# erthward/geonomics

Hardware: AMD Instinct MI355X
Metric: individual-timesteps/sec (higher is better)
Workload: dtype u64

## Files before the change

geonomics_amd/_native.py:

```python
import ctypes as C
import os

import numpy as np

_HERE = os.path.dirname(os.path.abspath(__file__))
LIB_PATH = os.environ.get('GNX_LIB') or os.path.join(_HERE, 'libgnxhip.so')

DIST = {'lognormal': 0, 'wald': 1, 'levy': 2}
MATE_UNIFORM, MATE_NEAREST, MATE_INVERSE = 0, 1, 2
SURF_NONE, SURF_MIXTURE, SURF_UNIMODAL = 0, 1, 2
(F_X, F_Y, F_AGE, F_SEX, F_ID, F_E, F_Z, F_FIT, F_GROW, F_GENO) = range(10)
(R_N, R_NPAIRS, R_K, R_D, R_COUNTS) = range(5)
KERNELS = ['move', 'sort', 'permute', 'find_mates', 'pairs', 'offspring',
           'crossover', 'phenotype', 'density', 'death', 'compact', 'crossover_tail']

EXPORTS = [
    'gnx_create', 'gnx_destroy', 'gnx_last_error', 'gnx_words_per_hom', 'gnx_blocks_per_hom',
    'gnx_set_stream', 'gnx_synchronize', 'gnx_upload_rasters',
    'gnx_upload_layer', 'gnx_set_species_params', 'gnx_upload_population',
    'gnx_init_population', 'gnx_set_recomb_paths', 'gnx_set_trait',
    'gnx_set_dominance', 'gnx_set_deleterious', 'gnx_upload_genomes',
    'gnx_assign_genomes', 'gnx_set_z', 'gnx_age', 'gnx_move',
    'gnx_pop_dynamics', 'gnx_pop_dynamics_mate', 'gnx_pop_dynamics_die',
    'gnx_set_z_range', 'gnx_step', 'gnx_counts', 'gnx_step_index',
# ... 377 lines not shown
        self._chk(self.lib.gnx_tile2_vt_counts(self.h, _ptr(cnt, C.c_int64)))
        return cnt

    def tile2_vt_bases(self, bases):
        b = _arr(bases, np.int64)
        assert b.size == 64
        self._chk(self.lib.gnx_tile2_vt_bases(self.h, _ptr(b, C.c_int64)))

    def step_begin(self, burn):
        self._chk(self.lib.gnx_step_begin(self.h, int(bool(burn))))

    def step_mid(self, burn, with_selection):
        self._chk(self.lib.gnx_step_mid(self.h, int(bool(burn)), int(bool(with_selection))))

    def step_end(self, burn):
        self._chk(self.lib.gnx_step_end(self.h, int(bool(burn))))

    def counts(self):
        n, b, d = C.c_int64(), C.c_int64(), C.c_int64()
        self._chk(self.lib.gnx_counts(self.h, C.byref(n), C.byref(b), C.byref(d)))
        return n.value, b.value, d.value

    def totals(self):
        out = np.zeros(6, np.int64)
        self._chk(self.lib.gnx_totals(self.h, _ptr(out, C.c_int64)))
        return dict(zip(('steps', 'ind_steps', 'births', 'deaths', 'xo_births', 'dd_steps'),
                        (int(v) for v in out)))

    def reset_totals(self):
        self._chk(self.lib.gnx_reset_totals(self.h))

    PATH_COUNTS = ('lazy_mortalities', 'xo_launch_p2', 'xo_flush', 'jobs_lanes_256',
                   'jobs_lanes_512', 'sort_hist_gather', 'gc_with_pending_xo', 'make_dense',
                   'moves_ahead')

    def path_counts(self):
        out = np.zeros(len(self.PATH_COUNTS), np.int64)
        n = self.lib.gnx_path_counts(self.h, _ptr(out, C.c_int64), len(out))
        assert n == len(out), 'gnx_path_counts: the library has %d counters' % n
        return dict(zip(self.PATH_COUNTS, (int(v) for v in out)))

    def reset_path_counts(self):
        self._chk(self.lib.gnx_reset_path_counts(self.h))

    @property
    def N(self):
        return self.counts()[0]

    @property
    def step_index(self):
        return self.lib.gnx_step_index(self.h)

    @step_index.setter
    def step_index(self, v):
        self._chk(self.lib.gnx_set_step_index(self.h, C.c_int64(int(v))))

    def synchronize(self):
        self._chk(self.lib.gnx_synchronize(self.h))

    def set_defer_crossover(self, on):
        self._chk(self.lib.gnx_set_defer_crossover(self.h, int(bool(on))))

    def set_crossover_overlap(self, mode):
        self._chk(self.lib.gnx_set_crossover_overlap(self.h, int(mode)))

    def debug_halves(self):
        out = np.zeros(6, np.int64)
# ... 1295 lines not shown
```

geonomics_amd/csrc/gnx_api.hip:

```cpp
#include <cmath>
#include <cstdarg>
#include <algorithm>
#include <atomic>
#include <chrono>
#include "gnx_internal.h"
#include "gnx_rng.h"
#include "gnx_compact.h"

static thread_local char g_err[1024] = "";

void gnx_set_error(const char* fmt, ...) {
  va_list ap;
  va_start(ap, fmt);
  vsnprintf(g_err, sizeof(g_err), fmt, ap);
  va_end(ap);
}

extern "C" const char* gnx_last_error(void) { return g_err; }

extern "C" int gnx_words_per_hom(int32_t L) {
  int w = (L + 63) / 64;
  return ((w + 15) / 16) * 16;
}

// ... 375 lines not shown
  GNXCHK(dalloc(&h->req_px, cap));
  GNXCHK(dalloc(&h->req_py, cap));
  GNXCHK(dalloc(&h->req_count, 1));
  h->blk_stride = (int)((cap + 1023) / 1024) + 2;
  GNXCHK(dalloc(&h->blk_cnt, (size_t)3 * h->blk_stride));
  GNXCHK(dalloc(&h->blk_off, (size_t)3 * h->blk_stride));
  GNXCHK(dalloc(&h->cnt_dev, 8));
  GNXCHK(dalloc(&h->tickets, 8));
  GNXCHK(dalloc(&h->nmax2, 2));
  HIPCHK(hipMemset(h->nmax2, 0, 2 * sizeof(unsigned long long)));
  HIPCHK(hipEventCreateWithFlags(&h->ev_pairs, gnx_order_event_flags()));
  HIPCHK(hipEventCreateWithFlags(&h->ev_latP, gnx_order_event_flags()));
  HIPCHK(hipEventCreateWithFlags(&h->ev_perm, gnx_order_event_flags()));
  HIPCHK(hipEventCreateWithFlags(&h->ev_binsN, gnx_order_event_flags()));
  HIPCHK(hipMemset(h->tickets, 0, 8 * sizeof(unsigned int)));
  HIPCHK(hipHostMalloc((void**)&h->h_pin, 32 * sizeof(int64_t),
                       hipHostMallocCoherent | hipHostMallocMapped));
  memset(h->h_pin, 0, 32 * sizeof(int64_t));
  HIPCHK(hipHostGetDevicePointer((void**)&h->h_pin_dev, h->h_pin, 0));
  if (cfg->L > 0) {
    for (int k = 0; k < 2; ++k) {
      HIPCHK(hipMalloc(&h->jobs[k], (size_t)cap * 2 * h->NB * 16));
      HIPCHK(hipMalloc(&h->jobs_bp[k], (size_t)cap * 2 * h->NB * 8));
      GNXCHK(dalloc(&h->n_jobs_dev[k], 1));
      HIPCHK(hipEventCreateWithFlags(&h->ev_xo_done[k], gnx_order_event_flags()));
      HIPCHK(hipEventCreateWithFlags(&h->ev_xo_wide[k], gnx_order_event_flags()));
    }
    HIPCHK(hipEventCreateWithFlags(&h->ev_jobs, gnx_order_event_flags()));
  }
  HIPCHK(hipEventCreateWithFlags(&h->ev_counts, hipEventDisableTiming));
  h->xo_launch_late = h->xo_launch_late_default = cap > gnx_dd_max_cap();
  h->compact_fill = gnx_env_int("GNX_COMPACT_FILL", 1) != 0;
  h->permute_split = gnx_env_int("GNX_PERMUTE_SPLIT", 1) != 0;
  *out = h;
  return 0;
}

extern "C" void gnx_destroy(gnx_state* h) {
  if (!h) return;
  host_marks_report();
  if (gnx_host_times() && g_host_steps > 0)
    fprintf(stderr, "[gnx host times] %lld steps: %.1f us/step in gnx_step, %.1f us of it waiting for counts\n",
            g_host_steps, 1e6 * g_host_step_s / g_host_steps, 1e6 * g_host_wait_s / g_host_steps);
  (void)gnx_xo_launch_pending(h);
  (void)hipStreamSynchronize(h->stream);
  gnx_dd_destroy(h);
  (void)gnx_comm_free(h);
  {
    void* vt[] = {h->vt_cls, h->vt_scls, h->vt_blk_nz, h->vt_rank, h->vt_pblk, h->vt_blk_cnt, h->vt_blk_off, h->vt_count, h->vt_base};
    for (void* q : vt)
      if (q) (void)hipFree(q);
  }
  if (h->stream2) (void)hipStreamSynchronize(h->stream2);
  if (h->stream3) (void)hipStreamSynchronize(h->stream3);
  for (int k = 0; k < 2; ++k) {
    (void)hipFree(h->jobs[k]);
    (void)hipFree(h->jobs_bp[k]);
    (void)hipFree(h->n_jobs_dev[k]);
    if (h->ev_xo_done[k]) (void)hipEventDestroy(h->ev_xo_done[k]);
    if (h->ev_xo_wide[k]) (void)hipEventDestroy(h->ev_xo_wide[k]);
  }
  if (h->ev_jobs) (void)hipEventDestroy(h->ev_jobs);
  if (h->ev_counts) (void)hipEventDestroy(h->ev_counts);
  for (int k = 0; k < 2; ++k) {
    free_soa(&h->soa[k]);
    (void)hipFree(h->key[k]);
// ... 580 lines not shown
  bool count;
  explicit GnxStepTimer(bool c) : count(c) {}
  ~GnxStepTimer() {
    if (gnx_host_times()) {
      g_host_step_s += std::chrono::duration<double>(std::chrono::steady_clock::now() - t0).count();
      if (count) ++g_host_steps;
    }
  }
};

extern "C" int gnx_step_begin(gnx_state* h, int32_t burn) {
  GNXCHK(need_params(h));
  GNXCHK(check_recomb_ready(h, burn != 0));
  GnxStepTimer timer(true);
  if (h->mort_wait || h->pairs_wait) {
    gnx_set_error("gnx_step_begin: the previous step of this handle was not finished (gnx_step_end)");
    return 1;
  }
  h->tot[0] += 1;
  h->tot[1] += h->N - h->n_ghost;
  h->last_xo_births = 0;
  h->step_burn = burn != 0;
  h->tile2_mode = false;
  if (h->moved_ahead) {
    GNXCHK(gnx_move_ahead_join(h));
  } else if (h->sp.move) {
    h->move_writes_keys = h->sp.mating_radius >= 0;
    int rc = gnx_l_move(h, true, nullptr, nullptr, nullptr, nullptr, true);
    h->move_writes_keys = false;
    GNXCHK(rc);
  } else {
    GNXCHK(gnx_l_age(h));
  }
  GNXCHK(gnx_l_sort_by_cell(h, true));
  int rc_pairs = gnx_l_find_pairs_enqueue(h, nullptr, true);
  GNXCHK(gnx_wait_permute_rest(h));
  return rc_pairs;
}

extern "C" int gnx_step_mid(gnx_state* h, int32_t burn, int32_t with_selection) {
  GnxStepTimer timer(false);
  int64_t P = 0, B = 0;
  GNXCHK(gnx_l_find_pairs_finish(h, &P));
  if (P > 0 && !h->spl_P.valid)
    GNXCHK(gnx_l_density(h, P, h->mid_x, h->mid_y, &h->spl_P, nullptr));
  GNXCHK(gnx_l_mate(h, burn != 0, false, 0, &B));
  h->last_births = B;
  GNXCHK(gnx_l_density_N(h));
  GNXCHK(gnx_l_death_probs(h, with_selection != 0 && !burn));
  return gnx_l_mortality_enqueue(h, nullptr);
}

extern "C" int gnx_step_end(gnx_state* h, int32_t burn) {
  GnxStepTimer timer(false);
  int64_t D = 0;
  GNXCHK(gnx_l_mortality_finish(h, &D));
  h->last_deaths = D;
  h->step += 1;
  h->tot[2] += h->last_births;
  h->tot[3] += h->last_deaths;
  if (!burn) h->tot[4] += h->last_xo_births;
  return 0;
}

extern "C" int gnx_step(gnx_state* h, int32_t burn, int32_t with_selection) {
  GNXCHK(gnx_step_begin(h, burn));
  GNXCHK(gnx_step_mid(h, burn, with_selection));
  return gnx_step_end(h, burn);
// ... 518 lines not shown
```

geonomics_amd/csrc/gnx_internal.h:

```cpp
#pragma once
#include <cstring>
#include <cstdint>
#include <cstdio>
#include <cstdlib>
#include <string>
#include <vector>
#include <utility>
#include <hip/hip_runtime.h>
#include "../../include/gnx_hip.h"
#include "gnx_half.h"

#define GNX_MAX_TRAITS 16
#define GNX_MAX_LAYERS 16
#define GNX_DISP_ATTEMPTS 8
#define GNX_SPARSE_MAX_BP 24

void gnx_set_error(const char* fmt, ...);

static inline int gnx_env_int(const char* name, int dflt) {
  const char* v = getenv(name);
  return v ? atoi(v) : dflt;
}
static inline int64_t gnx_dd_max_cap() {
  static const int64_t v = getenv("GNX_DD_MAX_CAP") ? atoll(getenv("GNX_DD_MAX_CAP")) : 600000;
// ... 181 lines not shown
  const int lane = threadIdx.x & 63;
  int idx = -1;
  while (todo) {
    const int leader = __ffsll((long long)todo) - 1;
    const int d = __shfl(dest, leader);
    const unsigned long long same = __ballot(dest == d);
    int base = 0;
    if (lane == leader) base = atomicAdd(&counts[d], (int)__popcll(same));
    base = __shfl(base, leader);
    if (dest == d) idx = base + (int)__popcll(same & ((1ull << lane) - 1ull));
    todo &= ~same;
  }
  return idx;
}
__device__ __forceinline__ int gnx_route_dest(const RouteGeo& g, int k, int orow, int oc, int cx, int cy) {
  if (k == 4) return (orow * g.C + oc) != g.me ? orow * g.C + oc : -1;
  const int rr = orow + k / 3 - 1, cc = oc + k % 3 - 1;
  if (rr >= 0 && rr < g.R && cc >= 0 && cc < g.C && cx >= g.cx0[cc] && cx <= g.cx1[cc] &&
      cy >= g.cy0[rr] && cy <= g.cy1[rr])
    return rr * g.C + cc;
  return -1;
}
#endif
enum {
  GNX_PC_LAZY_MORT = 0,
  GNX_PC_XO_P2,
  GNX_PC_XO_FLUSH,
  GNX_PC_JOBS_256,
  GNX_PC_JOBS_512,
  GNX_PC_SORT_GATHER,
  GNX_PC_GC_PENDING_XO,
  GNX_PC_MAKE_DENSE,
  GNX_PC_MOVE_AHEAD,
  GNX_PC_COUNT
};

struct gnx_state {
  gnx_config cfg{};
  gnx_species_params sp{};
  bool have_sp = false;
  hipStream_t stream = nullptr;
  hipStream_t stream2 = nullptr;
  bool xo_pending = false;
  bool own_stream = false;
  int W64 = 0;
  int64_t N = 0;
  int64_t max_id = -1;
  int64_t step = 0;
  int64_t last_births = 0, last_deaths = 0;
  int64_t tot[6]{};
  int64_t pc[GNX_PC_COUNT]{};
  int64_t n_ghost = 0;

  GnxSoA soa[2]{};
  int cur = 0;

  uint64_t* G = nullptr;
  int row_spread = 1;
  int32_t* free_rows = nullptr;
  int64_t n_free = 0;
  int32_t* hmap = nullptr;
  uint8_t* half_mark = nullptr;
  int32_t* half_free = nullptr;
  int32_t* half_top = nullptr;
  int64_t half_free_est = 0;
  int64_t gc_runs = 0;
// ... 231 lines not shown
  hipEvent_t ev_perm_rest = nullptr;
  bool fb_pending = false;
  const float *fbp_x = nullptr, *fbp_y = nullptr;
  int64_t fbp_N = 0;
  hipEvent_t ev_alive = nullptr;
  int32_t* fill_cnt = nullptr;
  hipEvent_t ev_fill = nullptr;
  int64_t fill_guess = 0;
  uint32_t* cell32 = nullptr;
  uint32_t* keyk[2]{};
  int32_t* valk[2]{};
  void* os_scratch = nullptr;
  uint32_t* os_ktmp = nullptr;
  int32_t* os_vtmp = nullptr;
  int32_t* ord_cnt = nullptr;
  int32_t* ord_off = nullptr;
  hipEvent_t ev_ord = nullptr;
  bool ord_inflight = false;
  bool keys_ordmode = false;
  bool keys_fresh = false;
  bool hist_fresh = false;
  bool holes = false;
  int64_t holes_N = 0;
  RouteGeo* route_geo_dev = nullptr;
  uint64_t route_geo_epoch = 0;
  bool move_counts_routes = false;
  bool move_counted_routes = false;
  bool tile_lazy_ok = false;
  int64_t holes_flagged = 0;
  bool eager_move = false;
  bool move_ahead_ok = false;
  bool moved_ahead = false;
  hipEvent_t ev_moved = nullptr;
  bool e_stale = false;
  bool move_writes_keys = false;
  int n_bin_blocks = 0;
  double* nodes = nullptr;
  double* K_over = nullptr;
  unsigned long long* nmax_bits = nullptr;
  double* p_death = nullptr;
  double* d_cell = nullptr;
  uint8_t* dead_in = nullptr;
  int32_t* counts_rast[2]{};
  int counts_cur = 0;
  bool counts_init = false;
  double* red = nullptr;

  int32_t* blk_cnt = nullptr;
  int32_t* blk_off = nullptr;
  int blk_stride = 0;
  int32_t* cnt_dev = nullptr;
  unsigned int* tickets = nullptr;

  int64_t* h_pin = nullptr;
  int64_t* h_pin_dev = nullptr;
  int64_t pin_seq = 0;
  void* h_stage = nullptr;
  size_t h_stage_bytes = 0;

  void* tile_comm = nullptr;
  GnxDD* dd = nullptr;
  GnxDDRec* dd_ring = nullptr;
  GnxDDRec* dd_ring_dev = nullptr;
  bool dd_active = false;
  int64_t dd_seq = 0;
  int64_t dd_seen = 0;
// ... 27 lines not shown
int gnx_half_reserve(gnx_state* h, int64_t blocks);
int gnx_gc(gnx_state* h);
static inline const int32_t* gnx_alias_bp(const gnx_state* h) {
  return (h->alias_xo && h->sparse_paths) ? h->bp_off : nullptr;
}
static inline const int32_t* gnx_alias_loci(const gnx_state* h) {
  return (h->alias_xo && h->sparse_paths) ? h->bp_loci : nullptr;
}

int gnx_publish(gnx_state* h, int slot, const int32_t* a, const int32_t* b = nullptr,
                const int32_t* c = nullptr, const int32_t* d = nullptr);

void gnx_time_begin(gnx_state* h, int kernel = -1);
void gnx_time_end(gnx_state* h, int kernel, double bytes);

int gnx_h2d(gnx_state* h, void* dst, const void* src, size_t bytes);
int gnx_d2h(gnx_state* h, void* dst, const void* src, size_t bytes);

int gnx_l_init_population(gnx_state* h, int64_t N);
int gnx_l_gather_e(gnx_state* h, int64_t first, int64_t n);
int gnx_l_age(gnx_state* h);
int gnx_l_move(gnx_state* h, bool inc_age, const float* inj_theta, const float* inj_dist,
               float* out_theta, float* out_dist, bool apply);
int gnx_l_move_ahead(gnx_state* h, int64_t N);
int gnx_move_ahead_join(gnx_state* h);
int gnx_l_sort_by_cell(gnx_state* h, bool split_rest = false);
int gnx_wait_permute_rest(gnx_state* h);
int gnx_permute_rest_launch(gnx_state* h);
int gnx_l_find_pairs(gnx_state* h, const uint8_t* d_keep, int64_t* n_pairs_out,
                     bool with_density = false);
int gnx_l_find_pairs_enqueue(gnx_state* h, const uint8_t* d_keep, bool with_density);
int gnx_l_find_pairs_finish(gnx_state* h, int64_t* n_pairs_out);
int gnx_l_births(gnx_state* h, int64_t* births_out);
int gnx_l_pair_cls(gnx_state* h, int64_t P, bool local);
int gnx_vt_buffers(gnx_state* h);
int gnx_l_mate(gnx_state* h, bool burn, bool inject, int64_t B_inject, int64_t* births_out,
               int64_t id_base = -1, bool tiled = false);
int gnx_l_dispersal_inject(gnx_state* h, int64_t B, int A, const float* d_mx, const float* d_my,
                           const float* d_theta, const float* d_dist, float* d_ox, float* d_oy,
                           int32_t* d_used);
int gnx_l_crossover_all(gnx_state* h, int64_t first_slot, int64_t B);
int gnx_l_crossover_requests(gnx_state* h, int64_t first_slot, int64_t n_req);
int gnx_l_crossover_pending(gnx_state* h, int64_t first_slot, int64_t B);
int gnx_l_crossover_survivors(gnx_state* h, int64_t first_slot, int64_t B, const int32_t* d_alive,
                              const int32_t* d_scan);
int gnx_xo_join(gnx_state* h);
int gnx_xo_flush_deferred(gnx_state* h);
int gnx_xo_launch_pending(gnx_state* h, int site = GNX_PC_XO_FLUSH);
int gnx_xo_wait_inflight(gnx_state* h);
int gnx_xo_prepare_jobs(gnx_state* h, int32_t** zero);
int gnx_xo_wait_wide(gnx_state* h);
double gnx_xo_bytes_per_birth(const gnx_state* h);
int gnx_l_rebuild_sel(gnx_state* h);
int gnx_l_path_sel(gnx_state* h);
int gnx_l_tb_from_rows(gnx_state* h, int64_t first, int64_t n, const int32_t* d_list,
                       const int64_t* d_slots, bool join = true);
int gnx_l_newborn_tb(gnx_state* h, int64_t first_slot, int64_t B);
int gnx_l_phenotype(gnx_state* h, int64_t first_slot, int64_t n, const int32_t* d_list = nullptr);
int gnx_l_assign_genomes(gnx_state* h, const int32_t* d_n_per_site);
int gnx_l_mutate(gnx_state* h, int n, const int64_t* d_slot, const int32_t* d_locus,
                 const uint8_t* d_hom);
int gnx_l_density(gnx_state* h, int64_t n, const float* d_x, const float* d_y, GnxSpline* spl,
                  const double* d_nodes_override, const int32_t* n_dev = nullptr);
struct GnxSetWords {
  int32_t* dst = nullptr;
  int32_t v[4] = {0, 0, 0, 0};
};
struct GnxPubWords {
  int n1 = 0;
  const int32_t* src1 = nullptr;
  int32_t* host1 = nullptr;
  int n2 = 0;
  const int32_t* src2 = nullptr;
  int32_t* host2 = nullptr;
};
int gnx_l_bins(gnx_state* h, int64_t n, const float* d_x, const float* d_y, const uint8_t* d_ghost,
               int32_t* d_bins, const int32_t* n_dev = nullptr, const GnxSetWords* sw = nullptr);
int gnx_l_spline(gnx_state* h, const int32_t* d_bins, GnxSpline* spl,
                 const double* d_nodes_override);
int gnx_l_spline_z(gnx_state* h, const int32_t* d_bins, GnxSpline* spl,
                   const double* d_nodes_override, bool housekeeping);
int gnx_l_raster(gnx_state* h, int which, double* d_out);
int gnx_l_density_N(gnx_state* h);
int gnx_l_lattice_P_async(gnx_state* h, int64_t n_max);
int gnx_bins_adults_launch(gnx_state* h);
void gnx_bins_adults_drop(gnx_state* h);
int gnx_l_bins_adults_async(gnx_state* h, const float* d_x, const float* d_y, int64_t N);
int gnx_wait_latP(gnx_state* h);
bool gnx_fused_bins(const gnx_state* h);
int gnx_l_death_probs(gnx_state* h, bool with_selection);
int gnx_l_mortality(gnx_state* h, const uint8_t* d_dead_inject, int64_t* deaths_out);
int gnx_l_mortality_enqueue(gnx_state* h, const uint8_t* d_dead_inject);
int gnx_l_mortality_finish(gnx_state* h, int64_t* deaths_out);
int gnx_l_spatial_diff(gnx_state* h, double* mean, double* sd, double* sums = nullptr);
int gnx_l_gather_genomes(gnx_state* h, int64_t n, const int64_t* d_slots, uint64_t* d_out);
int gnx_l_scatter_genomes(gnx_state* h, int64_t n, const uint64_t* d_in, int64_t first_slot);

int gnx_dd_l_sort(gnx_state* h, int32_t* d_bins, hipStream_t st);
int gnx_dd_l_pairs(gnx_state* h, int32_t* d_bins, hipStream_t st);
int gnx_dd_l_offspring(gnx_state* h, bool genomes, int32_t* d_bins, hipStream_t st);
int gnx_dd_l_density_N(gnx_state* h, int par, hipStream_t st);
int gnx_dd_l_death_probs(gnx_state* h, bool with_selection, int par, hipStream_t st);
int gnx_dd_l_alive(gnx_state* h, bool xo, int buf, hipStream_t st);
int gnx_dd_l_jobs(gnx_state* h, int buf, hipStream_t st);
int gnx_dd_l_crossover(gnx_state* h, int buf, hipStream_t st);
int gnx_dd_l_fill_lists(gnx_state* h, int has_rows, hipStream_t st);
int gnx_dd_l_fill(gnx_state* h, int has_rows, bool xo, hipStream_t st);
int gnx_dd_l_ord_end(gnx_state* h, int has_rows, bool xo, hipStream_t st);
bool gnx_dd_eligible(const gnx_state* h, bool burn);
int gnx_dd_leave(gnx_state* h);
void gnx_dd_destroy(gnx_state* h);

int gnx_block_scan(gnx_state* h, int K, int64_t n_items, const int32_t* cnt, int32_t* off,
                   int32_t* out, int64_t* host, int64_t seq = 0, hipStream_t st = nullptr,
                   const int32_t* extra = nullptr);
int gnx_os_hist_discard(gnx_state* h, hipStream_t st = nullptr);
bool gnx_l_lattices_tiled(gnx_state* h, bool have_pairs, const GnxPubWords& pub);
void gnx_host_mark(int id);
extern double g_host_step_s, g_host_wait_s;
bool gnx_host_times();
// ... 104 lines not shown
```

geonomics_amd/csrc/gnx_kernels_demog.hip:

```cpp
#include "gnx_internal.h"
#include <chrono>
#include "gnx_rng.h"
#include "gnx_compact.h"
#include "gnx_half.h"
#include "gnx_xo.h"

#define BIN_BLOCKS 512

__global__ void __launch_bounds__(256)
k_bins(int64_t n, const int32_t* n_dev, const float* x, const float* y, const uint8_t* ghost,
       double inv_hww, int nbx, int nby, int32_t* partials, GnxSetWords sw) {
  extern __shared__ int32_t lds_hist[];
  if (sw.dst && blockIdx.x == 0 && threadIdx.x < 4) sw.dst[threadIdx.x] = sw.v[threadIdx.x];
  if (n_dev) n = *n_dev;
  const int nb = nbx * nby;
  for (int k = threadIdx.x; k < nb; k += blockDim.x) lds_hist[k] = 0;
  __syncthreads();
  const int64_t stride = (int64_t)gridDim.x * blockDim.x;
  for (int64_t i = (int64_t)blockIdx.x * blockDim.x + threadIdx.x; i < n; i += stride) {
    if (ghost && ghost[i]) continue;
    int hx = min(nbx - 1, (int)floor((double)x[i] * inv_hww));
    int hy = min(nby - 1, (int)floor((double)y[i] * inv_hww));
    atomicAdd(&lds_hist[hy * nbx + hx], 1);
  }
// ... 599 lines not shown
}

static int launch_nmax(gnx_state* h) {
  if (!h->nmax_zeroed)
    HIPCHK(hipMemsetAsync(h->nmax_bits, 0, sizeof(unsigned long long), h->stream));
  h->nmax_zeroed = false;
  constexpr int GNX_NMAX_BLOCKS = 512;
  const int R = gnx_nmax_rows_fit(h->lat.Jx, 0);
  hipLaunchKernelGGL(k_nmax, dim3(std::min(h->cfg.H, GNX_NMAX_BLOCKS)), dim3(256),
                     gnx_nmax_lds_doubles(h->lat.Jx, R) * sizeof(double), h->stream,
                     make_splinec(h, h->spl_N), h->cfg.W, h->cfg.H, h->nmax_bits, R, gnx_nmax_scan_min());
  h->nmax_cur = h->nmax_bits;
  return 0;
}

constexpr int GNX_LATN_BLOCKS = 256;

bool gnx_fused_bins(const gnx_state* h) {
  const int64_t nn = (int64_t)h->lat.Jx * h->lat.Jy;
  const size_t lds = ((size_t)4 * nn + std::max(h->lat.Jx, h->lat.Jy) + 1 +
                      gnx_nmax_lds_doubles(h->lat.Jx, 1)) * sizeof(double);
  return !h->tiled && !h->tile2_mode && h->fb[0] != nullptr && h->stream3 != nullptr && lds <= 64 * 1024 &&
         (size_t)h->lat.nbx * h->lat.nby * sizeof(int32_t) <= 48 * 1024;
}

int gnx_wait_latP(gnx_state* h) {
  if (h->latP_inflight) {
    HIPCHK(hipStreamWaitEvent(h->stream, h->ev_latP, 0));
    h->latP_inflight = false;
  }
  return 0;
}

int gnx_l_lattice_P_async(gnx_state* h, int64_t n_max) {
  const GnxLattice& L = h->lat;
  const int64_t nn = (int64_t)L.Jx * L.Jy;
  const int nb = L.nbx * L.nby;
  const size_t lds_bytes = ((size_t)4 * nn + std::max(L.Jx, L.Jy) + 1) * sizeof(double);
  GNXCHK(gnx_wait_latP(h));
  HIPCHK(hipEventRecord(h->ev_pairs, h->stream));
  HIPCHK(hipStreamWaitEvent(h->stream3, h->ev_pairs, 0));
  GNXCHK(gnx_bins_adults_launch(h));
  if (!h->fb_zero[2])
    HIPCHK(hipMemsetAsync(h->fb[2], 0, (size_t)nb * sizeof(int32_t), h->stream3));
  const int blocks = (int)std::min<int64_t>(BIN_BLOCKS, std::max<int64_t>(1, (n_max + 255) / 256));
  hipLaunchKernelGGL(k_bins, dim3(blocks), dim3(256), (size_t)nb * sizeof(int32_t), h->stream3,
                     n_max, (const int32_t*)h->cnt_dev, (const float*)h->mid_x,
                     (const float*)h->mid_y, (const uint8_t*)nullptr, 1.0 / L.hww, L.nbx, L.nby,
                     h->fb[2], GnxSetWords{});
  hipLaunchKernelGGL(k_lattice, dim3(1), dim3(256), lds_bytes, h->stream3, L.Jx, L.Jy, L.nbx,
                     (const int32_t*)h->fb[2], L.areas, L.hww, L.cprime, h->spl_P.c,
                     (int32_t*)nullptr, 0, (unsigned long long*)nullptr, 1, 1);
  HIPCHK(hipEventRecord(h->ev_latP, h->stream3));
  HIPCHK(hipGetLastError());
  h->latP_inflight = true;
  h->fb_zero[2] = true;
  h->spl_P.valid = true;
  return 0;
}

int gnx_l_bins_adults_async(gnx_state* h, const float* d_x, const float* d_y, int64_t N) {
  if (!(h->have_sp && gnx_fused_bins(h))) {
    h->fb_adults = false;
    return 0;
  }
  const GnxLattice& L = h->lat;
  const int nb = L.nbx * L.nby;
  const int cur = h->fb_cur;
  if (!h->fb_zero[cur])
    HIPCHK(hipMemsetAsync(h->fb[cur], 0, (size_t)nb * sizeof(int32_t), h->stream));
  h->fbp_x = d_x;
  h->fbp_y = d_y;
  h->fbp_N = N;
  h->fb_pending = true;
  h->fb_zero[cur] = false;
  h->fb_adults = true;
  h->fb_count = N;
  return 0;
}

int gnx_bins_adults_launch(gnx_state* h) {
  if (!h->fb_pending) return 0;
  h->fb_pending = false;
  const GnxLattice& L = h->lat;
  const int nb = L.nbx * L.nby;
  const int64_t N = h->fbp_N;
  const int blocks = (int)std::min<int64_t>(BIN_BLOCKS, std::max<int64_t>(1, (N + 255) / 256));
  hipLaunchKernelGGL(k_bins, dim3(blocks), dim3(256), (size_t)nb * sizeof(int32_t), h->stream3, N,
                     (const int32_t*)nullptr, h->fbp_x, h->fbp_y, (const uint8_t*)nullptr,
                     1.0 / L.hww, L.nbx, L.nby, h->fb[h->fb_cur], GnxSetWords{});
  HIPCHK(hipEventRecord(h->ev_binsN, h->stream3));
  HIPCHK(hipGetLastError());
  h->binsN_inflight = true;
  return 0;
}

void gnx_bins_adults_drop(gnx_state* h) {
  if (h->fb_pending) {
    h->fb_pending = false;
    h->fb_adults = false;
  }
}

int gnx_l_density_N(gnx_state* h) {
  GnxSoA s = h->soa[h->cur];
  if (!(gnx_fused_bins(h) && h->fb_adults && h->fb_count == h->N)) {
    h->fb_adults = false;
    h->nmax_ready = false;
    h->last_N_fused = false;
    return gnx_l_density(h, h->N, s.x, s.y, &h->spl_N, nullptr);
// ... 1266 lines not shown
```

geonomics_amd/csrc/gnx_kernels_pop.hip:

```cpp
#include "gnx_internal.h"
#include "gnx_rng.h"
#include "gnx_compact.h"
#include "gnx_tb.h"
#include "gnx_bins.h"

static int gnx_id_bits(const gnx_state* h) {
  int b = 1;
  while (b < 40 && (h->max_id >> b) != 0) ++b;
  return b;
}
static bool gnx_ord_sort(const gnx_state* h) {
  return h->ord_mode && h->ord_valid && !h->tiled;
}

__device__ __forceinline__ int wave_min_i(int v) {
#pragma unroll
  for (int m = 32; m >= 1; m >>= 1) v = min(v, __shfl_xor(v, m));
  return v;
}
__device__ __forceinline__ int wave_max_i(int v) {
#pragma unroll
  for (int m = 32; m >= 1; m >>= 1) v = max(v, __shfl_xor(v, m));
  return v;
}
// ... 799 lines not shown
    if (h->sort64_tmp_bytes >= (size_t)n_sort * 12 && h->os_scratch) {
      GNXCHK(gnx_os_sort64_clean(h->os_scratch, h->sort64_tmp, h->key64[0], h->key64[1], h->perm[0],
                                 h->perm[1], (size_t)n_sort, idbits + cell_bits, h->stream));
      wipe_words = (int64_t)gnx_os_words_used64((size_t)n_sort, idbits + cell_bits);
    } else {
      GNXCHK(gnx_prim_sort64_bits(h->sort64_tmp, h->sort64_tmp_bytes, h->key64[0], h->key64[1],
                                  h->perm[0], h->perm[1], (size_t)n_sort, idbits + cell_bits,
                                  h->stream, alone));
    }
  }
  h->keys_fresh = false;
  gnx_time_end(h, GNX_K_SORT, (double)N * 40.0);
  gnx_time_begin(h);
  static const bool tile_split = gnx_env_int("GNX_TILE_SPLIT", 0) != 0;
  const bool split = split_rest && h->permute_split && (ordm ? !h->tiled : (tile_split && h->tile2_mode)) &&
                     h->stream3 != nullptr;
  hipLaunchKernelGGL(k_permute, dim3(gnx_grid(N, 256)), dim3(256), 0, h->stream, N, c.cap_inds,
                     ordm ? h->valk[1] : h->perm[1], a, b, c.n_layers, c.n_traits,
                     a.tb ? 2 * h->TW : 0, gnx_pair_seed(c.seed, h->step), h->tag, (uint4*)h->cand,
                     h->key64[1], idbits, h->cell_start, h->ncx * h->ncy,
                     ordm ? h->keyk[1] : nullptr, h->ord[h->ord_cur], h->ord_n,
                     h->ord[h->ord_cur ^ 1], h->perm[1], (uint4*)h->os_scratch, (wipe_words + 3) / 4,
                     split ? 1 : 0, (const GnxDD*)nullptr, GnxBinP{nullptr, 0.0, 0, 0},
                     h->id_order == 1 ? h->vt_count : (int32_t*)nullptr);
  if (split) {
    h->perm_rest_a = a;
    h->perm_rest_b = b;
    h->perm_rest_N = N;
    h->perm_rest_pending = true;
    GNXCHK(gnx_permute_rest_launch(h));
  }
  gnx_time_end(h, GNX_K_PERMUTE,
               (double)N * 2.0 * (33.0 + 4.0 * c.n_layers + 4.0 * c.n_traits + 16.0 * h->TW));
  GNXCHK(gnx_l_bins_adults_async(h, b.x, b.y, N));
  if (ordm) {
    h->ord_cur ^= 1;
    h->ord_n = N;
  } else if (h->ord_mode && !h->tiled) {
    if (h->ord_inflight) {
      HIPCHK(hipStreamWaitEvent(h->stream, h->ev_ord, 0));
      h->ord_inflight = false;
    }
    hipLaunchKernelGGL(k_iota, dim3(gnx_grid(N, 256)), dim3(256), 0, h->stream, N, h->perm[0]);
    GNXCHK(gnx_prim_sort64_bits(h->sort64_tmp, h->sort64_tmp_bytes, (const uint64_t*)b.id,
                                h->key64[0], h->perm[0], h->ord[h->ord_cur], (size_t)N, idbits,
                                h->stream, alone));
    h->ord_valid = true;
    h->ord_n = N;
  } else {
    h->ord_valid = false;
  }
  HIPCHK(hipGetLastError());
  h->cur ^= 1;
  if (h->tile_evict > 0) {
    const int64_t n = h->tile_evict;
    h->tile_evict = 0;
    h->N -= n;
    if (h->genomes_assigned && c.L > 0) {
      hipStream_t fs = h->stream;
      if (split) {
        GNXCHK(gnx_permute_rest_launch(h));
        fs = h->stream3;
      }
      hipLaunchKernelGGL(k_free_tail, dim3(gnx_grid(n, 256)), dim3(256), 0, fs, h->N, n,
                         h->soa[h->cur].grow, h->free_rows, h->n_free);
      if (split) HIPCHK(hipEventRecord(h->ev_perm_rest, h->stream3));
      h->n_free += n;
// ... 842 lines not shown
        const int wave = threadIdx.x >> 6;
        int before = vpre[vc[r]];
        for (int j = 0; j < r * 4 + wave; ++j) before += vcnt[j][vc[r]];
        vt.cls[p] = (uint8_t)vc[r];
        vt.rank[p] = before + vrw[r];
      }
    }
    if (bins.bins) gnx_bin_add(bins.bins, bin, f[r]);
  }
}

__global__ void k_panmixia(int64_t N, const int64_t* id, long long step, unsigned long long seed,
                           int32_t* focal, int32_t* mate) {
  int64_t i = (int64_t)blockIdx.x * blockDim.x + threadIdx.x;
  if (i >= N) return;
  uint4 r = gnx_rand4(seed, (unsigned long long)id[i], step, OP_PAIR_KEEP, 1);
  int f = (int)(((unsigned long long)r.x * (unsigned long long)N) >> 32);
  int m = (int)(((unsigned long long)r.y * (unsigned long long)N) >> 32);
  focal[i] = f;
  mate[i] = (m == f) ? -1 : m;
}

int gnx_l_find_pairs(gnx_state* h, const uint8_t* d_keep, int64_t* n_pairs_out, bool with_density) {
  int rc = gnx_l_find_pairs_enqueue(h, d_keep, with_density);
  if (rc) {
    *n_pairs_out = 0;
    return rc;
  }
  return gnx_l_find_pairs_finish(h, n_pairs_out);
}

constexpr int GNX_FM_EASY_ROUNDS = 2;

int gnx_l_find_pairs_enqueue(gnx_state* h, const uint8_t* d_keep, bool with_density) {
  int64_t N = h->N;
  h->n_pairs = 0;
  h->pairs_wait = false;
  if (N == 0) return 0;
  const gnx_species_params& sp = h->sp;
  GnxSoA s = h->soa[h->cur];
  int sexed = sp.sexed;
  const int32_t* focal = nullptr;
  gnx_time_begin(h);
  if (sp.mating_radius < 0) {
    focal = h->off_pair;
    hipLaunchKernelGGL(k_panmixia, dim3(gnx_grid(N, 256)), dim3(256), 0, h->stream, N, s.id,
                       h->step, h->cfg.seed, h->off_pair, h->mate);
  } else {
    float r = (float)sp.mating_radius;
    float r2 = r * r;
    FocalP fp{N, d_keep, (float)sp.b, sexed, sp.repro_age[0], h->step, h->cfg.seed};
    dim3 grid(gnx_grid(N, FM_PER_BLOCK)), blk(256);
    const uint4* cd = (const uint4*)h->cand;
    if (sp.mate_mode == GNX_MATE_NEAREST)
      hipLaunchKernelGGL(k_find_mates<GNX_MATE_NEAREST>, grid, blk, 0, h->stream, fp, s, cd,
                         h->inv_cs, h->cell_start, h->ncx, h->ncy, h->cell_ref, r, r2, GNX_FM_EASY_ROUNDS, h->mate);
    else if (sp.mate_mode == GNX_MATE_INVERSE)
      hipLaunchKernelGGL(k_find_mates<GNX_MATE_INVERSE>, grid, blk, 0, h->stream, fp, s, cd,
                         h->inv_cs, h->cell_start, h->ncx, h->ncy, h->cell_ref, r, r2, GNX_FM_EASY_ROUNDS, h->mate);
    else
      hipLaunchKernelGGL(k_find_mates<GNX_MATE_UNIFORM>, grid, blk, 0, h->stream, fp, s, cd,
                         h->inv_cs, h->cell_start, h->ncx, h->ncy, h->cell_ref, r, r2, GNX_FM_EASY_ROUNDS, h->mate);
  }
  gnx_time_end(h, GNX_K_FIND_MATES, (double)N * 16.0);
  GNXCHK(gnx_permute_rest_launch(h));
  gnx_time_begin(h);
  const int nb = (int)((N + GNX_CB - 1) / GNX_CB);
  PairP pp{N, focal, h->mate, d_keep, (float)sp.b, sexed, sp.repro_age[0], sp.repro_age[1],
           (sexed || sp.mating_radius < 0) ? 0 : 1,
           h->step, h->cfg.seed};
  GnxVtOut vto;
  GNXCHK(gnx_vt_out(h, &vto));
  hipLaunchKernelGGL(k_pair_flags, dim3(nb), dim3(256), 0, h->stream, pp, s, h->flag2, h->blk_cnt, vto);
  const int64_t seq = ++h->pin_seq;
  const bool with_top = h->half_top && h->genomes_assigned;
  hipLaunchKernelGGL(k_pair_compact, dim3(nb), dim3(256), 0, h->stream, N, focal, h->mate,
                     h->flag2, h->blk_off, s.x, s.y, h->key64[1], gnx_id_bits(h), h->pairs,
                     h->mid_x, h->mid_y, h->key64[0],
                     (const int32_t*)h->blk_cnt, h->cnt_dev,
                     h->h_pin_dev + 4, (long long)seq,
                     with_top ? (const int32_t*)h->half_top : (const int32_t*)nullptr,
                     (GnxDD*)nullptr, 0, (int64_t)0, GnxBinP{nullptr, 0.0, 0, 0}, vto);
  gnx_time_end(h, GNX_K_PAIRS, (double)N * 40.0);
  HIPCHK(hipGetLastError());
  if (with_density && gnx_fused_bins(h)) {
    GNXCHK(gnx_l_lattice_P_async(h, N));
  } else if (with_density) {
    const bool lds_bins = (size_t)h->lat.nbx * h->lat.nby * sizeof(int32_t) <= 48 * 1024;
    if (lds_bins)
      GNXCHK(gnx_l_density(h, N, h->mid_x, h->mid_y, &h->spl_P, nullptr, h->cnt_dev));
    else
      with_density = false;
  }
  h->pairs_wait = true;
  h->pairs_seq = seq;
  h->pairs_with_top = with_top;
  h->pairs_with_density = with_density;
  return 0;
}

int gnx_l_find_pairs_finish(gnx_state* h, int64_t* n_pairs_out) {
  *n_pairs_out = 0;
  if (!h->pairs_wait) return 0;
  h->pairs_wait = false;
  GNXCHK(gnx_wait_published(h, 4, h->pairs_seq));
  h->n_pairs = h->h_pin[4];
  if (h->pairs_with_top) h->half_free_est = h->h_pin[16];
  *n_pairs_out = h->n_pairs;
  if (!h->pairs_with_density) h->spl_P.valid = false;
  else if (h->n_pairs == 0) h->spl_P.valid = false;
  if (h->xo_launch_late) GNXCHK(gnx_xo_launch_pending(h, GNX_PC_XO_P2));
  return 0;
}

__global__ void k_births(int64_t P, const int32_t* pairs, const int64_t* id, float thr,
                         long long step, unsigned long long seed, int32_t* nb) {
  int64_t p = (int64_t)blockIdx.x * blockDim.x + threadIdx.x;
  if (p >= P) return;
  GnxStream st(seed, (unsigned long long)id[pairs[2 * p]], step, OP_BIRTHS);
// ... 9 lines not shown

__global__ void k_expand_births(int64_t P, const int32_t* nb, const int32_t* boff,
                                int32_t* off_pair) {
  int64_t p = (int64_t)blockIdx.x * blockDim.x + threadIdx.x;
  if (p >= P) return;
  int o = boff[p];
  for (int q = 0; q < nb[p]; ++q) off_pair[o + q] = (int32_t)p;
}

struct OffP {
  int64_t N, B, cap;
  int W, H, n_layers;
  float xmax, ymax, rrx, rry;
  int distr;
  float p1, p2;
  int surf, surf_layer;
  float surf_kappa;
  int sexed;
  float p_male;
  int fixed_nb;
  int genomes;
  int n_paths;
  int64_t id_base, n_free;
  long long step;
  unsigned long long seed;
  int fuse_tb, TW;
  const uint64_t* path_sel;
  const uint8_t* dom;
  GnxBinP bins;
  const GnxDD* dd;
  const uint64_t* ptb;
  const int32_t* pmap;
  const int32_t* P_dev;
};

struct GnxReq {
  int64_t* pid;
  int32_t* k;
  int32_t* key;
  uint8_t* start;
  float* px;
  float* py;
  int32_t* count;
};

__device__ __forceinline__ bool disperse_once(float mx, float my, float theta, float dist,
                                              float rrx, float rry, float xmax, float ymax,
                                              float& ox, float& oy) {
  float dx = cosf(theta) * dist;
  float dy = sinf(theta) * dist;
  if (rrx != 1.0f) dx *= rrx;
  if (rry != 1.0f) dy *= rry;
  ox = fminf(fmaxf(mx + dx, 0.0f), xmax);
  oy = fminf(fmaxf(my + dy, 0.0f), ymax);
  return ox > 0.0f && oy > 0.0f;
}

__global__ void __launch_bounds__(256)
k_offspring(OffP P, GnxSoA s, const float* rast, const int32_t* pairs, const int32_t* off_pair,
            const int32_t* boff, GnxGoff gf,
            int32_t* off_parent, int32_t* off_keys, uint8_t* off_start, GnxReq rq, GnxTraitTab T,
            int32_t* __restrict__ ord_tail) {
  int64_t k = (int64_t)blockIdx.x * blockDim.x + threadIdx.x;
  if (P.dd) {
    P.N = P.dd->N;
    P.B = P.dd->B;
    P.id_base = P.dd->max_id + 1;
    P.step = P.dd->step;
  }
  if (P.P_dev) {
    P.B = (int64_t)*P.P_dev * P.fixed_nb;
    if (P.N + P.B > P.cap || (P.genomes && P.B > P.n_free)) return;
  }
  if (k >= P.B) return;
  int64_t p, ord;
  if (P.fixed_nb > 0) {
    p = k / P.fixed_nb;
    ord = k - p * P.fixed_nb;
  } else {
    p = off_pair[k];
    ord = k - boff[p];
  }
  int64_t gk = k;
  if (gf.cls) {
    const int c = gf.cls[p];
    int64_t rk = gf.rank[p];
    if (gf.pblk) rk += gf.blk_off[(int64_t)gf.pblk[p] * GNX_VTN + c];
    gk = gf.vt_base[c] + rk * gf.mul + ord;
  } else if (gf.goff) {
    gk = gf.goff[p] + ord;
  }
  int i = pairs[2 * p], m = pairs[2 * p + 1];
  int64_t slot = P.N + k;
  unsigned long long oid = (unsigned long long)(P.id_base + gk);
  if (ord_tail) ord_tail[(P.dd ? P.N : 0) + gk] = (int32_t)slot;
  float mx = (s.x[i] + s.x[m]) / 2.0f;
  float my = (s.y[i] + s.y[m]) / 2.0f;
  const uint4 r = gnx_rand4(P.seed, oid, P.step, OP_OFFSPRING, 0);
  const uint8_t st0 = (uint8_t)(r.x & 1u), st1 = (uint8_t)((r.x >> 1) & 1u);
  const int32_t k0 = (int32_t)(((unsigned long long)r.y * (unsigned long long)P.n_paths) >> 32);
  const int32_t k1 = (int32_t)(((unsigned long long)r.z * (unsigned long long)P.n_paths) >> 32);
  const bool tb_regs = P.genomes && P.fuse_tb && P.TW > 0 && P.TW <= 2;
  uint64_t pi[4] = {0, 0, 0, 0}, pm[4] = {0, 0, 0, 0}, ps0[2] = {0, 0}, ps1[2] = {0, 0};
  const int64_t ip = P.pmap ? (int64_t)P.pmap[i] : (int64_t)i;
  const int64_t mp = P.pmap ? (int64_t)P.pmap[m] : (int64_t)m;
// ... 143 lines not shown
  OffP Q;
  Q.dd = nullptr;
  Q.N = h->N;
  Q.B = B;
  Q.cap = c.cap_inds;
  Q.W = c.W;
  Q.H = c.H;
  Q.n_layers = c.n_layers;
  Q.xmax = (float)(c.W - 0.001);
  Q.ymax = (float)(c.H - 0.001);
  Q.rrx = (float)sp.res_ratio[0];
  Q.rry = (float)sp.res_ratio[1];
  Q.distr = sp.disp_distr;
  Q.p1 = (float)sp.disp_p1;
  Q.p2 = (float)sp.disp_p2;
  Q.surf = sp.disp_surf;
  Q.surf_layer = sp.disp_surf_layer;
  Q.surf_kappa = (float)sp.disp_surf_kappa;
  Q.sexed = sp.sexed;
  Q.p_male = (float)sp.p_male;
  Q.fixed_nb = sp.n_births_fixed ? (int)sp.n_births_lambda : 0;
  Q.genomes = genomes ? 1 : 0;
  Q.n_paths = h->n_paths;
  Q.id_base = id_base >= 0 ? id_base : h->max_id + 1;
  Q.n_free = h->n_free;
  Q.step = h->step;
  Q.seed = c.seed;
  Q.fuse_tb = genomes ? 1 : 0;
  Q.TW = h->TW;
  Q.path_sel = h->path_sel;
  Q.dom = h->dom;
  Q.bins = GnxBinP{nullptr, 1.0 / h->lat.hww, h->lat.nbx, h->lat.nby};
  Q.P_dev = nullptr;
  Q.ptb = h->soa[h->cur].tb;
  Q.pmap = nullptr;
  return Q;
}

int gnx_l_mate(gnx_state* h, bool burn, bool inject, int64_t B_inject, int64_t* births_out,
               int64_t id_base, bool tiled) {
  const gnx_config& c = h->cfg;
  GnxSoA s = h->soa[h->cur];
  *births_out = 0;
  int64_t B = 0;
  bool ord_tail_used = false;
  GNXCHK(gnx_xo_flush_deferred(h));
  bool genomes = !burn && c.L > 0 && h->genomes_assigned;
  if (inject) {
    B = B_inject;
    if (B == 0) return 0;
    if (h->N + B > c.cap_inds || B > h->n_free) {
      gnx_set_error("capacity exceeded: N=%lld + B=%lld > cap_inds=%lld or free rows %lld",
                    (long long)h->N, (long long)B, (long long)c.cap_inds, (long long)h->n_free);
      return 2;
    }
    hipLaunchKernelGGL(k_offspring_inject, dim3(gnx_grid(B, 256)), dim3(256), 0, h->stream, h->N,
                       B, c.cap_inds, s, h->rast, c.n_layers, c.W, c.H, h->off_parent, h->max_id);
  } else {
    if (!tiled) {
      GNXCHK(gnx_l_births(h, &B));
      if (h->id_order == 1 && h->n_pairs > 0 && h->sp.mating_radius >= 0)
        GNXCHK(gnx_l_pair_cls(h, h->n_pairs, true));
    }
    B = h->n_births_pending;
    if (B == 0) {
      h->pair_goff_ready = false;
      return 0;
    }
    if (h->N + B > c.cap_inds || (genomes && B > h->n_free)) {
      gnx_set_error("capacity exceeded: N=%lld + births=%lld > cap_inds=%lld (free rows %lld)",
                    (long long)h->N, (long long)B, (long long)c.cap_inds, (long long)h->n_free);
      return 2;
    }
    OffP Q = gnx_make_offp(h, genomes, tiled, id_base, B);
    if (gnx_fused_bins(h) && h->fb_adults && h->fb_count == h->N) {
      Q.bins.bins = h->fb[h->fb_cur];
      h->fb_count += B;
    } else {
      h->fb_adults = false;
    }
    GnxReq rq{};
    if (tiled && genomes) {
      rq.pid = h->req_pid;
      rq.k = h->req_k;
      rq.key = h->req_key;
      rq.start = h->req_start;
      rq.px = h->req_px;
      rq.py = h->req_py;
      rq.count = h->req_count;
      if (!h->req_zeroed) HIPCHK(hipMemsetAsync(h->req_count, 0, sizeof(int32_t), h->stream));
      h->req_zeroed = false;
    }
    int32_t* ord_tail = nullptr;
    if (h->pair_goff_ready && h->pair_goff_local_base && h->ord_mode && h->ord_valid && !h->tiled &&
        h->ord_n == h->N)
      ord_tail = h->ord[h->ord_cur] + h->ord_n;
    ord_tail_used = ord_tail != nullptr;
    GnxGoff gf{};
    if (h->pair_goff_ready) gf = gnx_goff_vt(h);
    else if (tiled && !h->pair_goff_local) gf.goff = h->pair_goff;
    gnx_time_begin(h);
    hipLaunchKernelGGL(k_offspring, dim3(gnx_grid(B, 256)), dim3(256), 0, h->stream, Q, s, h->rast,
                       h->pairs, h->off_pair, h->boff, gf,
                       h->off_parent, h->off_keys, h->off_start, rq, gnx_trait_tab(h), ord_tail);
    gnx_time_end(h, GNX_K_OFFSPRING, (double)B * (60.0 + 8.0 * c.n_layers + 48.0 * h->TW +
                                                  4.0 * c.n_traits));
    if (tiled && genomes) {
      if (h->n_req_known >= 0) {
        h->n_req = h->n_req_known;
      } else {
        GNXCHK(gnx_publish(h, 0, h->req_count));
        HIPCHK(hipStreamSynchronize(h->stream));
        h->n_req = h->h_pin[0];
      }
    }
  }
  HIPCHK(hipGetLastError());
  if (genomes || inject) {
    const bool fused = !inject;
    if (!fused) GNXCHK(gnx_l_newborn_tb(h, h->N, B));
    const bool defer = h->defer_xo && !inject && h->stream2 != nullptr;
    if (defer) {
      if (tiled) GNXCHK(gnx_l_crossover_requests(h, h->N, h->n_req));
      h->xo_deferred = true;
      h->xo_first = h->N;
      h->xo_B = B;
    } else {
      GNXCHK(gnx_l_crossover_all(h, h->N, B));
    }
    if (c.n_traits > 0 && !tiled && !fused) GNXCHK(gnx_l_phenotype(h, h->N, B));
  }
  h->N += B;
  if (!tiled) h->max_id += B;
  if (h->pair_goff_ready) {
    h->pair_goff_ready = false;
    if (ord_tail_used)
      h->ord_n += B;
    else
      h->ord_valid = false;
// ... 110 lines not shown
```

Baseline: 2.601 billion.

## Enqueue offspring kernel speculatively before pair count is known on host

When births per pair are fixed, the offspring kernel is launched during find_pairs_enqueue with a grid sized to a bound derived from the previous step's births. The kernel reads the device pair count itself and exits if the count exceeds the bound. gnx_l_mate then skips its own launch when the actual birth count fits, which takes the offspring kernel off the host-synchronised critical path so it can overlap with host work. It adds consistency checks and a fallback launch when the bound is exceeded, and it reorders the bins, permute-wait and lattice-density launches so the speculative kernel's inputs are ready in time.

```diff
diff --git a/geonomics_amd/_native.py b/geonomics_amd/_native.py
--- a/geonomics_amd/_native.py
+++ b/geonomics_amd/_native.py
@@ -433,7 +433,7 @@
 
     PATH_COUNTS = ('lazy_mortalities', 'xo_launch_p2', 'xo_flush', 'jobs_lanes_256',
                    'jobs_lanes_512', 'sort_hist_gather', 'gc_with_pending_xo', 'make_dense',
-                   'moves_ahead')
+                   'moves_ahead', 'births_ahead', 'births_ahead_noop')
 
     def path_counts(self):
         out = np.zeros(len(self.PATH_COUNTS), np.int64)
diff --git a/geonomics_amd/csrc/gnx_api.hip b/geonomics_amd/csrc/gnx_api.hip
--- a/geonomics_amd/csrc/gnx_api.hip
+++ b/geonomics_amd/csrc/gnx_api.hip
@@ -431,6 +431,7 @@
   h->xo_launch_late = h->xo_launch_late_default = cap > gnx_dd_max_cap();
   h->compact_fill = gnx_env_int("GNX_COMPACT_FILL", 1) != 0;
   h->permute_split = gnx_env_int("GNX_PERMUTE_SPLIT", 1) != 0;
+  h->births_ahead = gnx_env_int("GNX_BIRTHS_AHEAD", 1) != 0;
   *out = h;
   return 0;
 }
@@ -1077,8 +1078,12 @@
   } else {
     GNXCHK(gnx_l_age(h));
   }
-  GNXCHK(gnx_l_sort_by_cell(h, true));
+  h->ba_want = true;
+  int rc_sort = gnx_l_sort_by_cell(h, true);
+  if (rc_sort) h->ba_want = false;
+  GNXCHK(rc_sort);
   int rc_pairs = gnx_l_find_pairs_enqueue(h, nullptr, true);
+  h->ba_want = false;
   GNXCHK(gnx_wait_permute_rest(h));
   return rc_pairs;
 }
diff --git a/geonomics_amd/csrc/gnx_internal.h b/geonomics_amd/csrc/gnx_internal.h
--- a/geonomics_amd/csrc/gnx_internal.h
+++ b/geonomics_amd/csrc/gnx_internal.h
@@ -237,6 +237,8 @@
   GNX_PC_GC_PENDING_XO,
   GNX_PC_MAKE_DENSE,
   GNX_PC_MOVE_AHEAD,
+  GNX_PC_BIRTHS_AHEAD,
+  GNX_PC_BIRTHS_AHEAD_NOOP,
   GNX_PC_COUNT
 };
 
@@ -534,6 +536,14 @@
   bool move_ahead_ok = false;
   bool moved_ahead = false;
   hipEvent_t ev_moved = nullptr;
+  bool births_ahead = true;
+  bool ba_want = false;
+  bool ba_launched = false;
+  bool ba_genomes = false;
+  bool ba_bins = false;
+  bool ba_ord_tail = false;
+  int64_t ba_bound = 0;
+  int64_t ba_N = 0;
   bool e_stale = false;
   bool move_writes_keys = false;
   int n_bin_blocks = 0;
@@ -627,6 +637,7 @@
 int gnx_l_find_pairs_enqueue(gnx_state* h, const uint8_t* d_keep, bool with_density);
 int gnx_l_find_pairs_finish(gnx_state* h, int64_t* n_pairs_out);
 int gnx_l_births(gnx_state* h, int64_t* births_out);
+int gnx_l_births_ahead(gnx_state* h, int64_t bound);
 int gnx_l_pair_cls(gnx_state* h, int64_t P, bool local);
 int gnx_vt_buffers(gnx_state* h);
 int gnx_l_mate(gnx_state* h, bool burn, bool inject, int64_t B_inject, int64_t* births_out,
@@ -677,10 +688,11 @@
                    const double* d_nodes_override, bool housekeeping);
 int gnx_l_raster(gnx_state* h, int which, double* d_out);
 int gnx_l_density_N(gnx_state* h);
-int gnx_l_lattice_P_async(gnx_state* h, int64_t n_max);
+int gnx_l_lattice_P_async(gnx_state* h, int64_t n_max, hipEvent_t after = nullptr);
 int gnx_bins_adults_launch(gnx_state* h);
 void gnx_bins_adults_drop(gnx_state* h);
-int gnx_l_bins_adults_async(gnx_state* h, const float* d_x, const float* d_y, int64_t N);
+int gnx_l_bins_adults_async(gnx_state* h, const float* d_x, const float* d_y, int64_t N,
+                            bool behind_rest = false);
 int gnx_wait_latP(gnx_state* h);
 bool gnx_fused_bins(const gnx_state* h);
 int gnx_l_death_probs(gnx_state* h, bool with_selection);
diff --git a/geonomics_amd/csrc/gnx_kernels_demog.hip b/geonomics_amd/csrc/gnx_kernels_demog.hip
--- a/geonomics_amd/csrc/gnx_kernels_demog.hip
+++ b/geonomics_amd/csrc/gnx_kernels_demog.hip
@@ -655,14 +655,17 @@
   return 0;
 }
 
-int gnx_l_lattice_P_async(gnx_state* h, int64_t n_max) {
+int gnx_l_lattice_P_async(gnx_state* h, int64_t n_max, hipEvent_t after) {
   const GnxLattice& L = h->lat;
   const int64_t nn = (int64_t)L.Jx * L.Jy;
   const int nb = L.nbx * L.nby;
   const size_t lds_bytes = ((size_t)4 * nn + std::max(L.Jx, L.Jy) + 1) * sizeof(double);
   GNXCHK(gnx_wait_latP(h));
-  HIPCHK(hipEventRecord(h->ev_pairs, h->stream));
-  HIPCHK(hipStreamWaitEvent(h->stream3, h->ev_pairs, 0));
+  if (!after) {
+    HIPCHK(hipEventRecord(h->ev_pairs, h->stream));
+    after = h->ev_pairs;
+  }
+  HIPCHK(hipStreamWaitEvent(h->stream3, after, 0));
   GNXCHK(gnx_bins_adults_launch(h));
   if (!h->fb_zero[2])
     HIPCHK(hipMemsetAsync(h->fb[2], 0, (size_t)nb * sizeof(int32_t), h->stream3));
@@ -682,7 +685,8 @@
   return 0;
 }
 
-int gnx_l_bins_adults_async(gnx_state* h, const float* d_x, const float* d_y, int64_t N) {
+int gnx_l_bins_adults_async(gnx_state* h, const float* d_x, const float* d_y, int64_t N,
+                            bool behind_rest) {
   if (!(h->have_sp && gnx_fused_bins(h))) {
     h->fb_adults = false;
     return 0;
@@ -690,6 +694,7 @@
   const GnxLattice& L = h->lat;
   const int nb = L.nbx * L.nby;
   const int cur = h->fb_cur;
+  const bool was_zero = h->fb_zero[cur];
   if (!h->fb_zero[cur])
     HIPCHK(hipMemsetAsync(h->fb[cur], 0, (size_t)nb * sizeof(int32_t), h->stream));
   h->fbp_x = d_x;
@@ -699,6 +704,7 @@
   h->fb_zero[cur] = false;
   h->fb_adults = true;
   h->fb_count = N;
+  if (behind_rest && was_zero && h->ba_want && h->births_ahead) GNXCHK(gnx_bins_adults_launch(h));
   return 0;
 }
 
diff --git a/geonomics_amd/csrc/gnx_kernels_pop.hip b/geonomics_amd/csrc/gnx_kernels_pop.hip
--- a/geonomics_amd/csrc/gnx_kernels_pop.hip
+++ b/geonomics_amd/csrc/gnx_kernels_pop.hip
@@ -855,7 +855,7 @@
   }
   gnx_time_end(h, GNX_K_PERMUTE,
                (double)N * 2.0 * (33.0 + 4.0 * c.n_layers + 4.0 * c.n_traits + 16.0 * h->TW));
-  GNXCHK(gnx_l_bins_adults_async(h, b.x, b.y, N));
+  GNXCHK(gnx_l_bins_adults_async(h, b.x, b.y, N, split));
   if (ordm) {
     h->ord_cur ^= 1;
     h->ord_n = N;
@@ -1764,10 +1764,13 @@
 
 constexpr int GNX_FM_EASY_ROUNDS = 2;
 
+static bool gnx_births_ahead_ok(gnx_state* h, const uint8_t* d_keep, int64_t* bound);
+
 int gnx_l_find_pairs_enqueue(gnx_state* h, const uint8_t* d_keep, bool with_density) {
   int64_t N = h->N;
   h->n_pairs = 0;
   h->pairs_wait = false;
+  h->ba_launched = false;
   if (N == 0) return 0;
   const gnx_species_params& sp = h->sp;
   GnxSoA s = h->soa[h->cur];
@@ -1804,6 +1807,9 @@
   GnxVtOut vto;
   GNXCHK(gnx_vt_out(h, &vto));
   hipLaunchKernelGGL(k_pair_flags, dim3(nb), dim3(256), 0, h->stream, pp, s, h->flag2, h->blk_cnt, vto);
+  int64_t ba_bound = 0;
+  const bool ba = gnx_births_ahead_ok(h, d_keep, &ba_bound);
+  if (ba) GNXCHK(gnx_wait_permute_rest(h));
   const int64_t seq = ++h->pin_seq;
   const bool with_top = h->half_top && h->genomes_assigned;
   hipLaunchKernelGGL(k_pair_compact, dim3(nb), dim3(256), 0, h->stream, N, focal, h->mate,
@@ -1815,8 +1821,15 @@
                      (GnxDD*)nullptr, 0, (int64_t)0, GnxBinP{nullptr, 0.0, 0, 0}, vto);
   gnx_time_end(h, GNX_K_PAIRS, (double)N * 40.0);
   HIPCHK(hipGetLastError());
+  hipEvent_t after_pairs = nullptr;
+  if (ba && h->xo_launch_late && h->xo_ready_buf >= 0) {
+    GNXCHK(gnx_xo_launch_pending(h, GNX_PC_XO_P2));
+    after_pairs = h->ev_jobs;
+  }
+  if (ba && !(with_density && gnx_fused_bins(h))) GNXCHK(gnx_l_births_ahead(h, ba_bound));
   if (with_density && gnx_fused_bins(h)) {
-    GNXCHK(gnx_l_lattice_P_async(h, N));
+    GNXCHK(gnx_l_lattice_P_async(h, N, after_pairs));
+    if (ba) GNXCHK(gnx_l_births_ahead(h, ba_bound));
   } else if (with_density) {
     const bool lds_bins = (size_t)h->lat.nbx * h->lat.nby * sizeof(int32_t) <= 48 * 1024;
     if (lds_bins)
@@ -1892,6 +1905,7 @@
   const uint64_t* ptb;
   const int32_t* pmap;
   const int32_t* P_dev;
+  int64_t B_bound;
 };
 
 struct GnxReq {
@@ -1930,7 +1944,7 @@
   }
   if (P.P_dev) {
     P.B = (int64_t)*P.P_dev * P.fixed_nb;
-    if (P.N + P.B > P.cap || (P.genomes && P.B > P.n_free)) return;
+    if (P.B > P.B_bound || P.B > (int64_t)gridDim.x * blockDim.x) return;
   }
   if (k >= P.B) return;
   int64_t p, ord;
@@ -2140,9 +2154,57 @@
   Q.dom = h->dom;
   Q.bins = GnxBinP{nullptr, 1.0 / h->lat.hww, h->lat.nbx, h->lat.nby};
   Q.P_dev = nullptr;
+  Q.B_bound = 0;
   Q.ptb = h->soa[h->cur].tb;
   Q.pmap = nullptr;
   return Q;
+}
+
+static int32_t* gnx_births_ord_tail(gnx_state* h) {
+  if (h->pair_goff_ready && h->pair_goff_local_base && h->ord_mode && h->ord_valid && !h->tiled &&
+      h->ord_n == h->N)
+    return h->ord[h->ord_cur] + h->ord_n;
+  return nullptr;
+}
+
+static bool gnx_births_ahead_ok(gnx_state* h, const uint8_t* d_keep, int64_t* bound) {
+  const gnx_species_params& sp = h->sp;
+  if (!h->births_ahead || !h->ba_want || d_keep || h->tiled || h->tile2_mode || h->n_ghost > 0 ||
+      h->xo_deferred || !sp.n_births_fixed || (int)sp.n_births_lambda < 1)
+    return false;
+  const int64_t nb = (int64_t)sp.n_births_lambda;
+  const int64_t B = h->last_births + h->last_births / 8 + 1024 * nb;
+  const bool genomes = !h->step_burn && h->cfg.L > 0 && h->genomes_assigned;
+  if (h->N + B > h->cfg.cap_inds || (genomes && B > h->n_free)) return false;
+  *bound = B;
+  return true;
+}
+
+int gnx_l_births_ahead(gnx_state* h, int64_t bound) {
+  const bool genomes = !h->step_burn && h->cfg.L > 0 && h->genomes_assigned;
+  if (h->id_order == 1 && h->sp.mating_radius >= 0) GNXCHK(gnx_l_pair_cls(h, -1, true));
+  OffP Q = gnx_make_offp(h, genomes, false, -1, bound);
+  Q.P_dev = h->cnt_dev;
+  Q.B_bound = bound;
+  h->ba_bins = gnx_fused_bins(h) && h->fb_adults && h->fb_count == h->N;
+  if (h->ba_bins) Q.bins.bins = h->fb[h->fb_cur];
+  int32_t* ord_tail = gnx_births_ord_tail(h);
+  GnxGoff gf{};
+  if (h->pair_goff_ready) gf = gnx_goff_vt(h);
+  gnx_time_begin(h);
+  hipLaunchKernelGGL(k_offspring, dim3(gnx_grid(bound, 256)), dim3(256), 0, h->stream, Q,
+                     h->soa[h->cur], h->rast, h->pairs, h->off_pair, h->boff, gf, h->off_parent,
+                     h->off_keys, h->off_start, GnxReq{}, gnx_trait_tab(h), ord_tail);
+  gnx_time_end(h, GNX_K_OFFSPRING, (double)h->last_births * (60.0 + 8.0 * h->cfg.n_layers +
+                                                             48.0 * h->TW + 4.0 * h->cfg.n_traits));
+  HIPCHK(hipGetLastError());
+  h->ba_launched = true;
+  h->ba_bound = bound;
+  h->ba_N = h->N;
+  h->ba_genomes = genomes;
+  h->ba_ord_tail = ord_tail != nullptr;
+  ++h->pc[GNX_PC_BIRTHS_AHEAD];
+  return 0;
 }
 
 int gnx_l_mate(gnx_state* h, bool burn, bool inject, int64_t B_inject, int64_t* births_out,
@@ -2171,6 +2233,17 @@
         GNXCHK(gnx_l_pair_cls(h, h->n_pairs, true));
     }
     B = h->n_births_pending;
+    bool born_ahead = false;
+    if (h->ba_launched) {
+      h->ba_launched = false;
+      if (tiled || h->ba_N != h->N || h->ba_genomes != genomes) {
+        gnx_set_error("internal: births enqueued ahead for another step (N %lld / %lld, genomes %d / %d)",
+                      (long long)h->ba_N, (long long)h->N, (int)h->ba_genomes, (int)genomes);
+        return 1;
+      }
+      born_ahead = B <= h->ba_bound;
+      if (!born_ahead) ++h->pc[GNX_PC_BIRTHS_AHEAD_NOOP];
+    }
     if (B == 0) {
       h->pair_goff_ready = false;
       return 0;
@@ -2199,20 +2272,27 @@
       if (!h->req_zeroed) HIPCHK(hipMemsetAsync(h->req_count, 0, sizeof(int32_t), h->stream));
       h->req_zeroed = false;
     }
-    int32_t* ord_tail = nullptr;
-    if (h->pair_goff_ready && h->pair_goff_local_base && h->ord_mode && h->ord_valid && !h->tiled &&
-        h->ord_n == h->N)
-      ord_tail = h->ord[h->ord_cur] + h->ord_n;
+    int32_t* ord_tail = gnx_births_ord_tail(h);
     ord_tail_used = ord_tail != nullptr;
     GnxGoff gf{};
     if (h->pair_goff_ready) gf = gnx_goff_vt(h);
     else if (tiled && !h->pair_goff_local) gf.goff = h->pair_goff;
-    gnx_time_begin(h);
-    hipLaunchKernelGGL(k_offspring, dim3(gnx_grid(B, 256)), dim3(256), 0, h->stream, Q, s, h->rast,
-                       h->pairs, h->off_pair, h->boff, gf,
-                       h->off_parent, h->off_keys, h->off_start, rq, gnx_trait_tab(h), ord_tail);
-    gnx_time_end(h, GNX_K_OFFSPRING, (double)B * (60.0 + 8.0 * c.n_layers + 48.0 * h->TW +
-                                                  4.0 * c.n_traits));
+    if (born_ahead) {
+      if (h->ba_bins != (Q.bins.bins != nullptr) || h->ba_ord_tail != ord_tail_used) {
+        gnx_set_error("internal: births enqueued ahead with other arguments (bins %d / %d, index %d / %d)",
+                      (int)h->ba_bins, (int)(Q.bins.bins != nullptr), (int)h->ba_ord_tail,
+                      (int)ord_tail_used);
+        return 1;
+      }
+    } else {
+      gnx_time_begin(h);
+      hipLaunchKernelGGL(k_offspring, dim3(gnx_grid(B, 256)), dim3(256), 0, h->stream, Q, s, h->rast,
+                         h->pairs, h->off_pair, h->boff, gf,
+                         h->off_parent, h->off_keys, h->off_start, rq, gnx_trait_tab(h), ord_tail);
+      gnx_time_end(h, GNX_K_OFFSPRING, (double)B * (60.0 + 8.0 * c.n_layers + 48.0 * h->TW +
+                                                    4.0 * c.n_traits));
+    }
+    gnx_host_mark(5);
     if (tiled && genomes) {
       if (h->n_req_known >= 0) {
         h->n_req = h->n_req_known;
```

Result: no change. 2.598 billion (-0.1%).
